# jolibrain/jolineedle

Hardware: AMD Instinct MI355X
Metric: glimpse-patches/sec (448px, seq-len 20) REINFORCE step (higher is better)
Workload: dtype f32; 1 GPU; configs[2]/[3]: REINFORCE rollout, gpt-nano + yolox-nano encoder, 448px, seq-len 20, --enable-stop, 64 agents/GPU x 1 GPU, 4480x4480 synthetic images, forced non-STOP actions (S=T); global_batch=64, seq_len=20

## Files before the change

jolineedle_amd/csrc/api_net.hip:

```cpp
#include <algorithm>
#include <cstring>

#include "jn_internal.h"

using namespace jnr;

extern "C"
__global__ void bn_eval_table_kernel(const float* __restrict__ gamma, const float* __restrict__ beta,
                                     const float* __restrict__ rmean, const float* __restrict__ rvar, ChanTab t0,
                                     ChanTab t1, int C, float eps) {
  const int c = blockIdx.x * blockDim.x + threadIdx.x;
  if (c >= C) return;
  const float sc = gamma[c] / sqrtf(rvar[c] + eps);
  const float sh = beta[c] - rmean[c] * sc;
  t0.sc[c] = sc; t0.sh[c] = sh; t0.fl[c] = 1.0f;
  if (t1.sc) { t1.sc[c] = sc; t1.sh[c] = sh; t1.fl[c] = 1.0f; }
}

extern "C"
__global__ void fill_kernel(float* p, float v, long long n) {
  const long long i = (long long)blockIdx.x * blockDim.x + threadIdx.x;
  if (i < n) p[i] = v;
}

// ... 16 lines not shown
static bool defer_tab_runs(const Net& net, const View& v, int N, ChanTab& t) {
  const int off = net.tab_off[v.buf] + v.coff;
  auto deferred = [&](int c) { return net.h_td_hw[off + c] > 0.0f && (double)N * net.h_td_hw[off + c] <= (double)JN_DEFER_MAX_M; };
  bool any = false;
  for (int c = 0; c < v.C && !any; ++c) any = deferred(c);
  if (!any) return false;
  int ns = 0;
  bool fits = true;
  for (int c = 0; c < v.C && fits;) {
    const int tc = off + c;
    const bool d = deferred(c);
    int e = c + 1;
    if (d) {
      while (e < v.C && net.h_td_src[off + e] == net.h_td_src[tc] + (e - c) && net.h_td_goff[off + e] == net.h_td_goff[tc] + (e - c) &&
             net.h_td_boff[off + e] == net.h_td_boff[tc] + (e - c) && net.h_td_hw[off + e] == net.h_td_hw[tc])
        ++e;
    } else {
      while (e < v.C && !deferred(e)) ++e;
    }
    if (ns == 4) { fits = false; break; }
    const ChanTab::Run run{c, e, d ? net.h_td_src[tc] : -1, net.h_td_goff[tc], net.h_td_boff[tc], net.h_td_hw[tc]};
    (ns == 0 ? t.r0 : ns == 1 ? t.r1 : ns == 2 ? t.r2 : t.r3) = run;
    ++ns;
    c = e;
  }
  t.nseg = fits ? ns : 0;
  return true;
}

static inline float* slot_save(const Net& net, int slot) { return net.save + (size_t)slot * 2 * net.stat_channels; }

StemSrc patch_src(const void* ptr, int P, long long sample_stride) {
  return StemSrc{ptr, nullptr, sample_stride ? sample_stride : 3LL * P * P, (long long)P * P, P};
}

int ensure_slots(jn_ctx* ctx, Net& net, int n_slots) {
  if (net.n_slots >= n_slots) return JN_OK;
  const int MB = ctx->cfg.max_batch;
  float *tab = nullptr, *save = nullptr;
  double* stats = nullptr;
  char* act = nullptr;
  int rc;
  if ((rc = dev_alloc(ctx, &act, (size_t)n_slots * net.per_image_floats * MB * act_esz(net)))) return rc;
  if ((rc = dev_alloc(ctx, &tab, (size_t)n_slots * 3 * net.tab_channels))) return rc;
  if ((rc = dev_alloc(ctx, &save, (size_t)n_slots * 2 * net.stat_channels))) return rc;
  if ((rc = dev_alloc(ctx, &stats, (size_t)n_slots * JN_NREP * 2 * net.stat_channels))) return rc;
  const int n_old = net.n_slots;
  if (n_old > 0) {
    JN_HIP(hipDeviceSynchronize());
    JN_HIP(hipMemcpy(act, net.act, (size_t)n_old * net.per_image_floats * MB * act_esz(net), hipMemcpyDeviceToDevice));
    JN_HIP(hipMemcpy(tab, net.tab, (size_t)n_old * 3 * net.tab_channels * sizeof(float), hipMemcpyDeviceToDevice));
    JN_HIP(hipMemcpy(save, net.save, (size_t)n_old * 2 * net.stat_channels * sizeof(float), hipMemcpyDeviceToDevice));
    JN_HIP(hipMemcpy(stats, net.stats, (size_t)n_old * JN_NREP * 2 * net.stat_channels * sizeof(double), hipMemcpyDeviceToDevice));
  }
  net.act = act; net.tab = tab; net.save = save; net.stats = stats; net.n_slots = n_slots;
  for (int sl = n_old; sl < n_slots; ++sl) {
    float* t = tab + (size_t)sl * 3 * net.tab_channels;
    const long long n = net.tab_channels;
    hipLaunchKernelGGL(fill_kernel, dim3((unsigned)((n + 255) / 256)), dim3(256), 0, 0, t, 1.0f, n);
    hipLaunchKernelGGL(fill_kernel, dim3((unsigned)((2 * n + 255) / 256)), dim3(256), 0, 0, t + n, 0.0f, 2 * n);
  }
  JN_HIP(hipGetLastError());
  JN_HIP(hipDeviceSynchronize());
  if (n_old == 0) net.eval_tab_dirty = true;
  return JN_OK;
}

int refresh_eval_table(jn_ctx* ctx, Net& net, hipStream_t s) {
  if (!net.eval_tab_dirty) return JN_OK;
  for (const Op& op : net.ops) {
    if (op.wslot < 0) continue;
    const ConvW& cw = net.convs[op.wslot];
    if (!cw.has_bn) continue;
    ChanTab t1{nullptr, nullptr, nullptr};
    if (op.alias.buf >= 0) t1 = view_tab(net, 0, op.alias);
    hipLaunchKernelGGL(bn_eval_table_kernel, dim3((cw.cout + 63) / 64), dim3(64), 0, s, cw.gamma_dev, cw.beta_dev,
                       cw.rmean_dev, cw.rvar_dev, view_tab(net, 0, op.out), t1, cw.cout, kBnEps);
  }
  JN_HIP(hipGetLastError());
  net.eval_tab_dirty = false;
  return JN_OK;
}

static void refresh_x3_planes(jn_ctx* ctx, Net& net, hipStream_t s) {
  if (net.x3_hi == 0) {
    size_t lo = ctx->arena_size, hi = 0;
    for (const Op& op : net.ops) {
      if (op.kind != OP_PW || op.wslot < 0) continue;
      const ConvW& cw = net.convs[op.wslot];
      if (!cw.w_dev) continue;
      const size_t o = (size_t)(cw.w_dev - ctx->params);
      lo = std::min(lo, o); hi = std::max(hi, o + (size_t)cw.cout * cw.cin);
    }
    net.x3_lo = lo / 8 * 8; net.x3_hi = hi > lo ? (hi + 7) / 8 * 8 : 0;
  }
  if (net.x3_hi > net.x3_lo && net.x3_dirty) {
    launch_w_split3(ctx->params + net.x3_lo, ctx->params_x3 + 3 * net.x3_lo, (long long)(net.x3_hi - net.x3_lo), s);
    net.x3_dirty = false;
  }
}

void mark_params_written(jn_ctx* ctx) {
  for (Net& net : ctx->nets) net.eval_tab_dirty = net.x3_dirty = true;
}

static View net_full_view(const Net& net, int buf) {
  View v; v.buf = buf; v.H = net.bufs[buf].H; v.W = net.bufs[buf].W; v.C = net.bufs[buf].C; v.coff = 0;
  return v;
}

static int ensure_defer_tables(jn_ctx* ctx, Net& net) {
  if (net.defer_built) return JN_OK;
  net.defer_built = true;
  if (!ctx->params || !defer_eligible(net)) return JN_OK;
  const int n_ops = net.n_backbone_ops < 0 ? (int)net.ops.size() : net.n_backbone_ops;
  const int TC = net.tab_channels, SC = net.stat_channels;
  std::vector<int> td_src(TC, -1), td_g(TC, 0), td_b(TC, 0), fd_g(SC, 0), fd_b(SC, 0), fd_t0(SC, 0), fd_t1(SC, -1);
  std::vector<float> td_hw(TC, 0.0f), fd_hw(SC, 0.0f);
  std::vector<float*> fd_rm(SC, nullptr), fd_rv(SC, nullptr);
  for (int oi = 0; oi < n_ops; ++oi) {
    const Op& op = net.ops[oi];
    if (op.wslot < 0) continue;
    const ConvW& cw = net.convs[op.wslot];
    const float hw = (float)(op.out.H * op.out.W);
    for (int j = 0; j < cw.cout; ++j) {
      const int i = cw.stat_off + j;
      const int g = (int)(cw.gamma_dev - ctx->params) + j, b = (int)(cw.beta_dev - ctx->params) + j;
      fd_hw[i] = hw; fd_g[i] = g; fd_b[i] = b; fd_rm[i] = cw.rmean_dev + j; fd_rv[i] = cw.rvar_dev + j;
      const View* vs[2] = {&op.out, op.alias.buf >= 0 ? &op.alias : nullptr};
      for (int k = 0; k < 2; ++k) {
        if (!vs[k]) continue;
        const int tc = net.tab_off[vs[k]->buf] + vs[k]->coff + j;
        (k == 0 ? fd_t0 : fd_t1)[i] = tc;
        td_src[tc] = i; td_hw[tc] = hw; td_g[tc] = g; td_b[tc] = b;
      }
    }
  }
  int rc;
  auto up = [&](auto** dst, const auto& host) -> int {
    using T = typename std::remove_reference<decltype(host[0])>::type;
    typename std::remove_const<T>::type* d = nullptr;
    if ((rc = dev_alloc(ctx, &d, host.size()))) return rc;
    JN_HIP(hipMemcpy(d, host.data(), host.size() * sizeof(T), hipMemcpyHostToDevice));
    *dst = d;
    return JN_OK;
  };
  if ((rc = up(&net.td_src, td_src)) || (rc = up(&net.td_goff, td_g)) || (rc = up(&net.td_boff, td_b)) || (rc = up(&net.td_hw, td_hw)) ||
      (rc = up(&net.fd_hw, fd_hw)) || (rc = up(&net.fd_goff, fd_g)) || (rc = up(&net.fd_boff, fd_b)) || (rc = up(&net.fd_t0, fd_t0)) ||
      (rc = up(&net.fd_t1, fd_t1)) || (rc = up(&net.fd_rm, fd_rm)) || (rc = up(&net.fd_rv, fd_rv)))
    return rc;
  net.h_td_hw.assign(TC, 0.0f);
  for (int tc = 0; tc < TC; ++tc) if (td_src[tc] >= 0) net.h_td_hw[tc] = td_hw[tc];
  net.h_td_src = td_src; net.h_td_goff = td_g; net.h_td_boff = td_b;
  net.defer_ok = true;
  return JN_OK;
}

namespace {
struct OpProfile {
  std::vector<hipEvent_t> ev;
  hipStream_t s;
  double tot_us = 0, tot_b = 0;
  OpProfile(bool on, int n_events, hipStream_t s_) : s(s_) {
    if (on) { ev.resize(n_events); for (auto& e : ev) (void)hipEventCreate(&e); }
  }
  ~OpProfile() { for (auto& e : ev) (void)hipEventDestroy(e); }
  explicit operator bool() const { return !ev.empty(); }
  void mark(int i) { if (!ev.empty()) (void)hipEventRecord(ev[i], s); }
  void row(const Op& op, int from, int to, double bytes, bool bwd) {
    static const char* kn[] = {"stem", "pw", "dw", "conv3", "spp", "upsample", "addact", "pred"};
    float ms = 0;
    (void)hipEventElapsedTime(&ms, ev[from], ev[to]);
    tot_us += ms * 1e3; tot_b += bytes;
    fprintf(stderr, "%-8s %-44s in %3dx%3dx%3d out %3dx%3dx%3d s%d", kn[op.kind], op.name.c_str(), op.in.H, op.in.W, op.in.C,
            op.out.H, op.out.W, op.out.C, op.stride);
    if (bwd) fprintf(stderr, " acc %d  %8.1f us  %8.1f MB  %6.0f GB/s\n", (int)op.acc_in, ms * 1e3, bytes / 1e6, bytes / (ms * 1e-3) / 1e9);
    else fprintf(stderr, "  %8.1f us  %7.1f MB  %7.0f GB/s\n", ms * 1e3, bytes / 1e6, bytes / (ms * 1e-3) / 1e9);
  }
  void total() { fprintf(stderr, "# total %.1f us, %.1f MB, %.0f GB/s\n", tot_us, tot_b / 1e6, tot_b / (tot_us * 1e-6) / 1e9); }
};
}

static void invalidate_slot_state(jn_ctx* ctx, int ni, int slot) {
  if (ni == ctx->enc_net) {
    if (slot == 0) ctx->sup_valid = false;
    else if (ni != JN_NET_DETECTOR || slot < det_slot_base(ctx)) ctx->train_out_valid = false;
  }
  if (ni == JN_NET_DETECTOR && slot >= det_slot_base(ctx) && slot - det_slot_base(ctx) < (int)ctx->det_pass.size())
    ctx->det_pass[slot - det_slot_base(ctx)].valid = false;
}

int run_net(jn_ctx* ctx, int ni, int N, const StemSrc& ss, int slot, int train, const int* skip_flag, int skip_when,
            hipStream_t s, bool with_head, int first_op) {
  Net& net = ctx->nets[ni];
  const int MB = ctx->cfg.max_batch;
  int rc;
  invalidate_slot_state(ctx, ni, slot);
  if (!train && (rc = refresh_eval_table(ctx, net, s))) return rc;
  const bool x3 = ctx->params_x3 && !std::getenv("JN_NO_PW_X3");
  if (x3) refresh_x3_planes(ctx, net, s);
  double* stats = train ? slot_stats(net, slot) : nullptr;
  float* save = train ? slot_save(net, slot) : nullptr;
  if (train && !ctx->stats_prezeroed) JN_HIP(hipMemsetAsync(stats, 0, (size_t)JN_NREP * 2 * net.stat_channels * sizeof(double), s));
  const long long rep_stride = 2LL * net.stat_channels;
  if (train && !with_head && (rc = ensure_defer_tables(ctx, net))) return rc;
  const bool defer = train && !with_head && net.defer_ok;
  std::vector<FwdStep> plan;
  if ((rc = plan_forward(net, N, train != 0, with_head, first_op, defer, plan))) return rc;
  const int n_ops = first_op + (int)plan.size();
  auto ptr = [&](const View& v) { return view_ptr(net, slot, MB, v); };
  auto tab = [&](const View& v) {
    ChanTab t = view_tab(net, slot, v);
    if (defer && defer_tab_runs(net, v, N, t)) {
      const int off = net.tab_off[v.buf] + v.coff;
      t.dsrc = net.td_src + off; t.dhw = net.td_hw + off; t.dgoff = net.td_goff + off; t.dboff = net.td_boff + off;
      t.dparams = ctx->params; t.dstats = stats; t.drep_stride = rep_stride; t.dN = N; t.dmax = JN_DEFER_MAX_M;
    }
    return t;
  };
  auto ld = [&](const View& v) { return net.bufs[v.buf].C; };
  auto finalize = [&](const Op& op, const ConvW& cw, bool deferred) {
    if (!train || !cw.has_bn || deferred) return;
    ChanTab t1{nullptr, nullptr, nullptr};
    if (op.alias.buf >= 0) t1 = tab(op.alias);
    launch_bn_finalize(stats + 2 * cw.stat_off, rep_stride, (double)N * op.out.H * op.out.W, cw.gamma_dev, cw.beta_dev,
                       defer ? nullptr : cw.rmean_dev, defer ? nullptr : cw.rvar_dev, defer ? nullptr : save + 2 * cw.stat_off,
                       tab(op.out), t1, cw.cout, kBnEps, kBnMomentum, skip_flag, skip_when, s);
  };
  static const bool layer_profile = std::getenv("JN_LAYER_PROFILE") != nullptr;
  OpProfile prof(layer_profile, n_ops + 1, s);
  prof.mark(first_op);
  std::vector<char> up_done(n_ops, 0);
  for (int oi = first_op; oi < n_ops; ++oi) {
    const Op& op = net.ops[oi];
    const FwdStep& st = plan[oi - first_op];
    switch (st.route) {
      case FR_STEM: {
        const ConvW& cw = net.convs[op.wslot];
        StemArgs a{ss.src, ss.positions, ss.pos_stride, ss.sample_stride, ss.chan_stride, ss.row_stride, net.P, N, cw.cout,
                   cw.w_dev, ptr(op.out), ld(op.out), net.act_dtype, train ? stats + 2 * cw.stat_off : nullptr, rep_stride,
                   skip_flag, skip_when, st.deferred ? JN_NREP_DEFER : JN_NREP, ss.src_u8};
        launch_stem(a, s);
        finalize(op, cw, st.deferred);
        break;
      }
      case FR_DWPW:
      case FR_DWPW_ADD: {
        const Op& nx = net.ops[st.link];
        DwPwArgs f{};
        f.in = ptr(op.in); f.in_ld = ld(op.in); f.itab = tab(op.in); f.w_dw = net.convs[op.wslot].w_dev; f.mtab = tab(op.out);
        f.w_pw = net.convs[nx.wslot].w_dev; f.out = ptr(nx.out); f.out_ld = ld(nx.out); f.dtype = net.act_dtype;
        f.C = op.out.C; f.cout = nx.out.C; f.N = N; f.H = op.in.H; f.W = op.in.W; f.OH = op.out.H; f.OW = op.out.W;
        f.stride = op.stride; f.skip_flag = skip_flag; f.skip_when = skip_when;
        if (st.route == FR_DWPW_ADD) {
          const Op& ad = net.ops[st.add];
          f.res = ptr(ad.res); f.res_ld = ld(ad.res); f.rtab = tab(ad.res); f.ptab = tab(nx.out);
          f.out = ptr(ad.out); f.out_ld = ld(ad.out);
        }
        launch_dwpw(f, s);
        break;
      }
      case FR_CONV: {
        const ConvW& cw = net.convs[op.wslot];
        ConvArgs a{};
        a.in = ptr(op.in); a.in_ld = ld(op.in); a.in_dtype = net.act_dtype; a.itab = tab(op.in); a.w = cw.w_dev;
        a.w_bf16 = cw.w_bf16;
        if (x3 && op.kind == OP_PW && (cw.w_dev - ctx->params) % 8 == 0) a.w_x3 = ctx->params_x3 + 3 * (cw.w_dev - ctx->params);
        a.bias = cw.b_dev; a.out = ptr(op.out); a.out_ld = ld(op.out); a.out_dtype = net.act_dtype;
        a.bf16_mfma = net.act_dtype == JN_BF16;
        a.N = N; a.H = op.in.H; a.W = op.in.W; a.OH = op.out.H; a.OW = op.out.W;
        a.cin = op.in.C; a.cout = op.out.C; a.stride = op.stride; a.act = op.act;
        a.stats = (train && cw.has_bn) ? stats + 2 * cw.stat_off : nullptr;
        a.stats_rep_stride = rep_stride;
        a.stats_nrep = st.deferred ? JN_NREP_DEFER : JN_NREP;
        a.skip_flag = skip_flag; a.skip_when = skip_when;
        if (st.link >= 0 && pw_fused_upsample_supported(a)) {
          const Op& up = net.ops[st.link];
          a.up_out = ptr(up.out); a.up_ld = ld(up.out); up_done[st.link] = 1;
        }
        if (op.kind == OP_PW) { JN_CHECK(launch_pw(a, s) == 0, JN_ESTATE, "1x1 conv %s: no kernel for this shape", op.name.c_str()); }
        else if (op.kind == OP_DW) launch_dw(a, s); else launch_conv3(a, s);
        finalize(op, cw, st.deferred);
        break;
// ... 420 lines not shown
```

jolineedle_amd/csrc/jn_internal.h:

```cpp
#pragma once
#include <hip/hip_runtime.h>

#include <cstdint>
#include <cstdio>
#include <map>
#include <string>
#include <vector>

#include "../../include/jnroll.h"
#include "jn_kernels.h"

namespace jnr {

void set_error(const char* fmt, ...);

#define JN_HIP(call)                                                                      \
  do {                                                                                    \
    hipError_t e_ = (call);                                                               \
    if (e_ != hipSuccess) {                                                               \
      jnr::set_error("%s failed: %s (%s:%d)", #call, hipGetErrorString(e_), __FILE__, __LINE__); \
      return JN_EHIP;                                                                     \
    }                                                                                     \
  } while (0)

#define JN_CHECK(cond, code, ...)   \
  do {                              \
    if (!(cond)) {                  \
      jnr::set_error(__VA_ARGS__);   \
      return (code);                \
    }                               \
  } while (0)

struct Buf {
  int H = 0, W = 0, C = 0;
  size_t per_image() const { return (size_t)H * W * C; }
};

struct View {
  int buf = -1;
  int H = 0, W = 0;
  int C = 0;
  int coff = 0;
};

enum OpKind {
  OP_STEM = 0,
  OP_PW,
  OP_DW,
  OP_CONV3,
  OP_SPP,
  OP_UPSAMPLE,
  OP_ADDACT,
  OP_PRED,
};

struct Op {
  OpKind kind;
  View in, out;
  View res;
  View alias;
  int stride = 1;
  int act = ACT_SILU;
  int wslot = -1;
  int level = 0, anchor0 = 0;
  bool acc_in = false;
  bool acc_res = false;
  std::string name;
};

struct ConvW {
  std::string prefix;
  std::string prefix2;
  int cout_first = 0;
  int cin = 0, cout = 0, k = 1, groups = 1;
  bool has_bn = true;
  bool has_bias = false;
  float* w_dev = nullptr;
  void* w_bf16 = nullptr;
  float* b_dev = nullptr;
  float *gamma_dev = nullptr, *beta_dev = nullptr;
  float *rmean_dev = nullptr, *rvar_dev = nullptr;
  int stat_off = 0;
};

struct Net {
  std::string prefix;
  bool depthwise = false;
  float depth = 0, width = 0;
  int P = 0;
  std::vector<Buf> bufs;
  std::vector<Op> ops;
  std::vector<ConvW> convs;
  View fpn[3];
  int n_backbone_ops = -1;
  size_t x3_lo = 0, x3_hi = 0;
  bool x3_dirty = true;
  int n_anchors = 0, head_hid = 0;
  float* pred_w[3] = {nullptr, nullptr, nullptr};
  float* pred_b[3] = {nullptr, nullptr, nullptr};
  size_t per_image_floats = 0;
  std::vector<size_t> buf_off;
  std::vector<int> tab_off;
  int tab_channels = 0;
  int stat_channels = 0;
  int n_slots = 0;
  int act_dtype = 0;
  char* act = nullptr;
  float* tab = nullptr;
  float* save = nullptr;
  double* stats = nullptr;
  int g_slots = 0;
  float* gact = nullptr;
  double* bred = nullptr;
  float* bconsts = nullptr;
  bool eval_tab_dirty = true;
  bool defer_ok = false, defer_built = false;
  int *td_src = nullptr, *td_goff = nullptr, *td_boff = nullptr; float* td_hw = nullptr;
  float* fd_hw = nullptr; int *fd_goff = nullptr, *fd_boff = nullptr, *fd_t0 = nullptr, *fd_t1 = nullptr;
  float **fd_rm = nullptr, **fd_rv = nullptr;
  std::vector<float> h_td_hw;
  std::vector<int> h_td_src, h_td_goff, h_td_boff;
};

enum BwdRoute {
  BR_NONE = 0,
  BR_PW_FUSED, BR_PW_FUSED_HALVES,
  BR_DW_FUSED, BR_STEM_FUSED,
  BR_PW, BR_DW, BR_STEM, BR_CONV3_S1, BR_CONV3_S2,
  BR_ADDACT_COPY, BR_ADDACT_FOLD,
  BR_SPP, BR_UPSAMPLE,
};
struct BwdStep {
  BwdRoute route = BR_NONE;
  View g;
  int red_by = 0;
  int red_in = -1, red_half = -1, red_in2 = -1, red_half2 = -1, red_split = 0;
  bool red2 = false;
  int fold = -1;
};
int plan_backward(const Net& net, bool with_head, int fpn_zero, std::vector<BwdStep>& plan);

enum FwdRoute {
  FR_NONE = 0,
  FR_STEM, FR_CONV,
  FR_DWPW, FR_DWPW_ADD,
  FR_ABSORBED,
  FR_SPP, FR_UPSAMPLE, FR_ADDACT, FR_PRED,
};
struct FwdStep {
  FwdRoute route = FR_NONE;
  int link = -1;
  int add = -1;
  bool deferred = false;
};
bool defer_eligible(const Net& net);
int plan_forward(const Net& net, int N, bool train, bool with_head, int first_op, bool defer, std::vector<FwdStep>& plan);

struct ParamEntry {
  jn_param_info info;
};
void add_param(std::vector<ParamEntry>& params, const std::string& name, std::initializer_list<int64_t> shape, int dtype,
               bool buffer, bool used);

struct ParamSeg {
  std::string name;
  int kind = 0, d0 = 0, d1 = 0, d2 = 0;
  size_t off = 0, numel = 0;
};

struct GptW {
  float *wte = nullptr, *wpe = nullptr, *embed_class = nullptr;
  float *proj_wt = nullptr, *proj_b = nullptr;
  float *pos1d = nullptr;
  float *pos2d_col = nullptr, *pos2d_row = nullptr;
  float *efpn_w = nullptr;
  float *efpn_lin_wt = nullptr, *efpn_lin_b = nullptr;
  float *head_wt = nullptr;
  float *lnf_w = nullptr, *lnf_b = nullptr;
  struct Layer {
// ... 175 lines not shown
```

jolineedle_amd/csrc/jn_kernels.h:

```cpp
#pragma once
#include <hip/hip_runtime.h>

#include <cstdint>

#include "../../include/jnroll.h"

namespace jnr {

enum { ACT_NONE = 0, ACT_SILU = 1, ACT_RELU = 2, ACT_SIGMOID = 3 };
enum { JN_F32 = 0, JN_BF16 = 1 };

constexpr int JN_NREP = 32;
constexpr int JN_WPART_MAX = 16384;

struct ChanTab {
  float* sc; float* sh; float* fl;
  const int* dsrc;
  const float* dhw;
  const int* dgoff; const int* dboff;
  const float* dparams;
  const double* dstats;
  long long drep_stride;
  int dN;
  long long dmax;
  struct Run { int c0, c1, stat0, g0, b0; float hw; };
  int nseg;
  Run r0, r1, r2, r3;
};
constexpr long long JN_DEFER_MAX_M = 65536;
constexpr int JN_NREP_DEFER = 8;

struct SlotBatch {
  int n = 1;
  long long act = 0;
  long long grad = 0;
  long long tab = 0;
  long long save = 0;
  long long red = 0;
  long long consts = 0;
  long long pos = 0;
};

struct StemArgs {
  const void* src; const int64_t* positions; int pos_stride;
  long long sample_stride, chan_stride; int row_stride;
  int P, N, cout;
  const float* w; void* out; int out_ld; int out_dtype;
  double* stats;
  long long stats_rep_stride;
  const int* skip_flag; int skip_when;
  int stats_nrep;
  int src_u8;
};

struct ConvArgs {
  const void* in; int in_ld; int in_dtype; ChanTab itab;
  const float* w; const float* bias;
  const void* w_bf16;
  void* out; int out_ld; int out_dtype;
  int bf16_mfma;
  int N, H, W, OH, OW, cin, cout, stride, act;
  int accumulate;
  int w_transposed;
  int in_identity;
  double* stats; long long stats_rep_stride;
  int stats_nrep;
  const int* skip_flag; int skip_when;
  int n_slots;
  long long in_slot_stride, out_slot_stride, tab_slot_stride;
  const void* w_x3;
  void* up_out; int up_ld;
};

struct DwPwArgs {
  const void* in; int in_ld; ChanTab itab; const float* w_dw; ChanTab mtab; const float* w_pw;
  void* out; int out_ld; int dtype; int C, cout, N, H, W, OH, OW, stride;
  const int* skip_flag; int skip_when;
  const void* res; int res_ld; ChanTab rtab;
  ChanTab ptab;
};
bool dwpw_supported(int C, int cout, int stride);
int launch_dwpw(const DwPwArgs& a, hipStream_t s);
int launch_stem(const StemArgs& a, hipStream_t s);
bool stem_rows_aligned(const StemArgs& a);
int launch_dw(const ConvArgs& a, hipStream_t s);
int launch_pw(const ConvArgs& a, hipStream_t s);
bool pw_fused_upsample_supported(const ConvArgs& a);
bool pw_res_supported(const ConvArgs& a);
int launch_pw_dir(const ConvArgs& a, int ctw, hipStream_t s);
int launch_pw_wide(const ConvArgs& a, hipStream_t s);
bool pw_xs_supported(const ConvArgs& a);
int launch_pw_xs(const ConvArgs& a, int pt, hipStream_t s, int wg_per_cu = 0);
int launch_pw_x3(const ConvArgs& a, int pt, hipStream_t s, int wg_per_cu = 0);
bool pw_x3_preferred(const ConvArgs& a);
bool pw_x3_bwd_data_supported(int cout, int cin);
int launch_pw_x3_bwd_data(const ConvArgs& a, const float* w, void* w3t, hipStream_t s);
bool pw_x1_supported(const ConvArgs& a);
int launch_pw_x1(const ConvArgs& a, hipStream_t s);
void launch_w_split3(const float* w, void* w3, long long n_floats, hipStream_t s);
int launch_spp(void* cat, int dtype, int ld, int h, int H, int W, int N, ChanTab it, const int* skip_flag,
               int skip_when, hipStream_t s);
int launch_upsample(const void* in, int in_ld, void* out, int out_ld, int dtype, int C, int H, int W, int N,
                    const int* skip_flag, int skip_when, hipStream_t s);
int launch_addact(const void* z, int z_ld, ChanTab zt, const void* res, int res_ld, ChanTab rt, void* out, int out_ld,
                  int dtype, int C, long long M, const int* skip_flag, int skip_when, hipStream_t s);
int launch_bn_finalize(const double* stats, long long rep_stride, double count, const float* gamma, const float* beta, float* run_mean,
                       float* run_var, float* save, ChanTab t0, ChanTab t1, int C, float eps, float momentum,
                       const int* skip_flag, int skip_when, hipStream_t s);
struct BnAllArgs {
  const double* stats; long long rep_stride; int n_stat; int N;
  const float* hw;
  const int* goff; const int* boff;
  const float* params;
  const int* t0; const int* t1;
  float* tab; int tab_channels;
  float* save;
  float* const* run_mean; float* const* run_var;
  float eps, momentum;
  const int* skip_flag; int skip_when;
  long long defer_max_m;
};
int launch_bn_finalize_all(const BnAllArgs& a, hipStream_t s);
int launch_nhwc_to_nchw(const void* in, int dtype, int in_ld, ChanTab it, float* out, int C, int HW, int N,
                        hipStream_t s);
int launch_efpn_linear(const float* e, const float* wt, float* part, int N, int K, int Co, int KS,
                       const int* skip_flag, int skip_when, hipStream_t s);

int launch_conv3(const ConvArgs& a, hipStream_t s);
int launch_conv3_bwd_data_s2(const float* gz, int g_ld, const float* w, float* gin, int gin_ld, int H, int W, int OH,
                             int OW, int Co, int Ci, int N, int accumulate, hipStream_t s,
                             const SlotBatch& sb = SlotBatch{});
int launch_conv3_bwd_weight(const float* gz, int g_ld, const void* x, int x_dtype, int x_ld, ChanTab it, float* gw, int H,
                            int W, int OH, int OW, int Co, int Ci, int N, int stride, hipStream_t s,
                            const SlotBatch& sb = SlotBatch{});
int launch_head_pred(const void* reg, int reg_ld, ChanTab rt, const void* cls, int cls_ld, ChanTab ct, int dtype,
                     const float* wp, const float* bp, float* raw, int hid, int Hl, int Wl, int stride, int A, int a0,
                     int N, hipStream_t s, int logits_only = 0);
int launch_det_scatter(const float* boxes, const int* counts, float* out_boxes, int* out_counts, int B, int cols, int col,
                       int K, const int* skip_flag, int skip_when, hipStream_t s);
int launch_postprocess(const float* raw, int A, int N, float conf, float nms_thr, float clamp_max, float* boxes,
                       int* counts, int max_out, int* stats, hipStream_t s);

struct DetGeom { int A; int a0[3]; int H[3]; int W[3]; int stride[3]; };
int launch_yolox_loss(const float* raw, const float* labels, int N, int nb, const DetGeom& geo, float* d_raw, float* acc,
                      int use_l1, float loss_scale, float* metrics, float* scale, hipStream_t s);
int launch_head_pred_bwd(const float* d_raw, const float* scale, const void* reg, int reg_ld, ChanTab rt, const void* cls,
                         int cls_ld, ChanTab ct, int dtype, const float* wp, float* g_reg, float* g_cls, float* g_wp,
                         float* g_bp, int hid, int HW, int A, int a0, int N, hipStream_t s);

int launch_bn_bwd_reduce(const float* g, int g_ld, const void* z, int z_dtype, int z_ld, ChanTab t, const float* save,
                         int C, long long M, double* red_out, long long rep_stride, hipStream_t s,
                         const SlotBatch& sb = SlotBatch{});
int launch_bn_bwd_consts(const double* red, long long rep_stride, double count, const float* gamma, const float* beta,
                         const float* save, float* consts, float* g_gamma, float* g_beta, int C, hipStream_t s,
                         const SlotBatch& sb = SlotBatch{}, int raw_moment = 0);
int launch_bn_bwd_gz(float* g, int g_ld, const void* z, int z_dtype, int z_ld, ChanTab t, const float* save,
                     const float* consts, int C, long long M, hipStream_t s, const SlotBatch& sb = SlotBatch{});
int launch_pw_bwd_weight(const float* gz, int g_ld, const void* x, int x_dtype, int x_ld, ChanTab it, float* gw,
                         float* wpart, long long M, int N, int K, hipStream_t s, const SlotBatch& sb = SlotBatch{},
                         long long gz_slot_stride = -1);
int launch_wpart_reduce(float* gw, float* wpart, int n, hipStream_t s);
struct PwBwdFusedArgs {
  const float* g; int g_ld;
  const float* z; int z_ld; ChanTab ot;
  const float* save; const float* consts;
  const float* x; int x_ld; ChanTab it;
  const float* w;
  float* gx; int gx_ld; int accumulate;
  float* gw; float* wpart;
  long long M; int cout, cin;
  SlotBatch sb;
  double* red_in; long long red_rep_stride; double* red_in2; int red_split;
  const float* gadd; int gadd_ld;
  const float* red2_z; int red2_ld; const float* red2_sc; const float* red2_sh;
};
struct DwBwdFusedArgs {
// ... 181 lines not shown
```

jolineedle_amd/csrc/kernels_pwxs.hip:

```cpp
#include <hip/hip_runtime.h>

#include <algorithm>
#include <cstdlib>

#include "jn_kernels.h"
#include "jn_reduce.h"
#include "jn_tab.h"
#include "jn_types.h"

namespace jnr {

struct UpsDst { float* out; int ld; int W; int HW; };
template <bool UPS>
__device__ __forceinline__ void ups_store(const UpsDst& u, long long m, int n, const f32x4& v) {
  if constexpr (UPS) {
    const long long img = m / u.HW;
    const int rem = (int)(m - img * u.HW), y = rem / u.W, x = rem - y * u.W;
    float* d = u.out + ((img * 2 * (u.HW / u.W) + 2 * y) * (2LL * u.W) + 2 * x) * u.ld + n;
    *reinterpret_cast<f32x4*>(d) = v;
    *reinterpret_cast<f32x4*>(d + u.ld) = v;
    d += 2LL * u.W * u.ld;
    *reinterpret_cast<f32x4*>(d) = v;
    *reinterpret_cast<f32x4*>(d + u.ld) = v;
  }
// ... 134 lines not shown
static void launch_pw_xs_t(const ConvArgs& a, long long M, int wg_per_cu, hipStream_t s) {
  constexpr int BM = 16 * PT;
  const size_t smem = ((size_t)BM * (K + 8) + 3 * K) * sizeof(float);
  auto kern = pw_xs_kernel<K, CTW, PT, D, UPS>;
  static int places = 0;
  if (!places) {
    (void)hipFuncSetAttribute(reinterpret_cast<const void*>(kern), hipFuncAttributeMaxDynamicSharedMemorySize, 160 * 1024);
    int per_cu = 0;
    if (hipOccupancyMaxActiveBlocksPerMultiprocessor(&per_cu, reinterpret_cast<const void*>(kern), 256, smem) != hipSuccess || per_cu < 1) per_cu = 1;
    places = per_cu;
  }
  const long long n_tiles = (M + BM - 1) / BM;
  const int per_cu = std::max(1, std::min(places, wg_per_cu > 0 ? wg_per_cu : 2));
  const long long gx = std::min<long long>(n_tiles, 256LL * per_cu);
  hipLaunchKernelGGL(kern, dim3((unsigned)gx), dim3(256), smem, s, (const float*)a.in, a.in_ld, a.itab, a.w, (float*)a.out,
                     a.out_ld, M, a.stats, a.stats_rep_stride, a.stats_nrep > 0 ? a.stats_nrep : JN_NREP, a.skip_flag,
                     a.skip_when, UpsDst{(float*)a.up_out, a.up_ld, a.W, a.H * a.W});
}

bool pw_xs_supported(const ConvArgs& a) {
  if (a.bf16_mfma || a.in_dtype != JN_F32 || a.out_dtype != JN_F32 || a.bias || a.act != ACT_NONE || a.w_transposed ||
      a.accumulate || a.n_slots > 1)
    return false;
  const int K = a.cin, N = a.cout;
  if (!(K == 64 || K == 128 || K == 256 || K == 512) || !(N == 64 || N == 128 || N == 256)) return false;
  if (K == 64 && N == 256) return false;
  if (K == 512 && N != 256) return false;
  if (K == 256 && N == 64) return false;
  return a.in_ld % 4 == 0 && a.out_ld % 4 == 0;
}

int launch_pw_xs(const ConvArgs& a, int pt, hipStream_t s, int wg_per_cu) {
  if (!pw_xs_supported(a)) return -1;
  const long long M = (long long)a.N * a.H * a.W;
  const int K = a.cin, ctw = a.cout / 64;
  if (pt == 0) {
    const bool big = K == 512 || (K == 64 && ctw == 2);
    pt = big ? 4 : 2;
    if (wg_per_cu == 0) wg_per_cu = big ? 1 : 2;
  }
  if (a.up_out) {
    if (!(K == 256 && ctw == 2 && pt == 2)) return -1;
    launch_pw_xs_t<256, 2, 2, 4, true>(a, M, wg_per_cu, s);
    return 0;
  }
#define JN_XS(K_, C_, D_)                                                          \
  if (K == K_ && ctw == C_) {                                                      \
    if (pt == 4) launch_pw_xs_t<K_, C_, 4, D_>(a, M, wg_per_cu, s); else launch_pw_xs_t<K_, C_, 2, D_>(a, M, wg_per_cu, s); \
    return 0;                                                                      \
  }
  JN_XS(64, 1, 4) JN_XS(64, 2, 4)
  JN_XS(128, 1, 8) JN_XS(128, 2, 8) JN_XS(128, 4, 2)
  JN_XS(256, 2, 4) JN_XS(256, 4, 2)
  JN_XS(512, 4, 2)
#undef JN_XS
  return -1;
}


__global__ __launch_bounds__(256) void w_split3_kernel(const float* __restrict__ w, bf16_t* __restrict__ w3, long long n8) {
  const long long i = (long long)blockIdx.x * 256 + threadIdx.x;
  if (i >= n8) return;
  const f32x4 a = *reinterpret_cast<const f32x4*>(w + 8 * i), b = *reinterpret_cast<const f32x4*>(w + 8 * i + 4);
  bf16x8 h, m, l;
#pragma unroll
  for (int e = 0; e < 8; ++e) {
    const float v = e < 4 ? a[e] : b[e - 4];
    const bf16_t vh = (bf16_t)v;
    const float r1 = v - (float)vh;
    const bf16_t vm = (bf16_t)r1;
    const float r2 = r1 - (float)vm;
    h[e] = vh; m[e] = vm; l[e] = (bf16_t)r2;
  }
  bf16x8* o = reinterpret_cast<bf16x8*>(w3 + 24 * i);
  o[0] = h; o[1] = m; o[2] = l;
}

void launch_w_split3(const float* w, void* w3, long long n_floats, hipStream_t s) {
  const long long n8 = n_floats / 8;
  if (n8 <= 0) return;
  hipLaunchKernelGGL(w_split3_kernel, dim3((unsigned)((n8 + 255) / 256)), dim3(256), 0, s, w, (bf16_t*)w3, n8);
}

struct SlotSpan { int n_slots; long long in, out; };
template <int K, int CTW, int PT, int D, int NP, typename XT, bool UPS = false, bool SLOTS = false>
__global__ __launch_bounds__(256, (K <= 64 ? 3 : CTW <= 2 ? 2 : 1)) void pw_x3_kernel(
    const XT* __restrict__ x, int x_ld, ChanTab it, const bf16_t* __restrict__ w3, XT* __restrict__ out, int out_ld,
    long long M, double* __restrict__ stats, long long rep_stride, int nrep, const int* __restrict__ skip_flag,
    int skip_when, UpsDst ups, SlotSpan sl) {
  if (skip_flag && *skip_flag >= skip_when) return;
  constexpr int BM = 16 * PT, LDK = K + 16, KQ = K / 4, NJ = K / 32, N = 64 * CTW;
  constexpr int NX = BM * KQ / 256;
  constexpr int NXB = NX < 16 ? NX : 16;
  static_assert(256 % KQ == 0 && NX >= 1 && NX % NXB == 0 && NJ % D == 0, "pw_x3 tile mapping");
  extern __shared__ __attribute__((aligned(16))) unsigned char smem_raw[];
  bf16_t* Xp = reinterpret_cast<bf16_t*>(smem_raw);
  float* Tb = reinterpret_cast<float*>(Xp + NP * BM * LDK);
  const int tid = threadIdx.x, lane = tid & 63, wave = tid >> 6;
  const int lm = lane & 15, g = lane >> 4;
  const long long tiles_per_slot = (M + BM - 1) / BM;
  const long long n_tiles = SLOTS ? tiles_per_slot * sl.n_slots : tiles_per_slot;

  const bf16_t* wrow[CTW];
#pragma unroll
  for (int c = 0; c < CTW; ++c)
    wrow[c] = SLOTS ? w3 + (long long)(wave * CTW + c) * (K / 32) * 3 * 512 + lane * 8
                    : w3 + ((long long)((wave * CTW + c) * 16 + lm) * (K / 8) + g) * 24;
  auto wfrag = [&](int c, int j, int t) -> bf16x8 {
    if constexpr (SLOTS) return *reinterpret_cast<const bf16x8*>(wrow[c] + (j * 3 + t) * 512);
    else return *reinterpret_cast<const bf16x8*>(wrow[c] + 96 * j + 8 * t);
  };
  bf16x8 wr[D][CTW][NP];
#pragma unroll
  for (int u = 0; u < D; ++u)
#pragma unroll
    for (int c = 0; c < CTW; ++c)
#pragma unroll
      for (int t = 0; t < NP; ++t) wr[u][c][t] = wfrag(c, u, t);

  const int q = tid % KQ, r0 = tid / KQ;
  constexpr int RS = 256 / KQ;
  f32x4 xr[NXB];
  const XT* xs = x;
  auto fetch = [&](long long m0, int b) {
#pragma unroll
    for (int u = 0; u < NXB; ++u) {
      long long m = m0 + r0 + (long long)(b * NXB + u) * RS;
      m = m < M ? m : M - 1;
      xr[u] = ld4(xs + m * x_ld + 4 * q);
    }
  };
  auto locate = [&](long long t) -> long long {
    if constexpr (SLOTS) {
      const long long slot = t / tiles_per_slot;
      xs = x + slot * sl.in;
      return (t - slot * tiles_per_slot) * BM;
    } else {
      return t * BM;
    }
  };
  long long tile = blockIdx.x;
  long long m0 = locate(tile);
  fetch(m0, 0);
  tab_to_lds(Tb, K, K, it, tid, 256);
  __syncthreads();
  const f32x4 sc = *reinterpret_cast<const f32x4*>(Tb + 4 * q), sh = *reinterpret_cast<const f32x4*>(Tb + K + 4 * q),
              fl = *reinterpret_cast<const f32x4*>(Tb + 2 * K + 4 * q);
  f32x4 s1[CTW], s2[CTW];
#pragma unroll
  for (int c = 0; c < CTW; ++c) { s1[c] = f32x4{0.f, 0.f, 0.f, 0.f}; s2[c] = s1[c]; }

#pragma unroll 1
  for (; tile < n_tiles; tile += gridDim.x) {
    XT* outs = out;
    if constexpr (SLOTS) outs = out + (tile / tiles_per_slot) * sl.out;
#pragma unroll
    for (int b = 0; b < NX / NXB; ++b) {
      if (b > 0) fetch(m0, b);
#pragma unroll
      for (int u = 0; u < NXB; ++u) {
        const int r = r0 + (b * NXB + u) * RS;
        f32x4 v = tf4_tab(xr[u], sc, sh, fl);
        if (m0 + r >= M) v = f32x4{0.f, 0.f, 0.f, 0.f};
        const bf16x4 vh = __builtin_convertvector(v, bf16x4);
        bf16_t* dst = Xp + r * LDK + 4 * q;
        *reinterpret_cast<bf16x4*>(dst) = vh;
        if constexpr (NP == 3) {
          const f32x4 r1 = v - __builtin_convertvector(vh, f32x4);
          const bf16x4 vm = __builtin_convertvector(r1, bf16x4);
          const f32x4 r2 = r1 - __builtin_convertvector(vm, f32x4);
          const bf16x4 vl = __builtin_convertvector(r2, bf16x4);
          *reinterpret_cast<bf16x4*>(dst + BM * LDK) = vm;
          *reinterpret_cast<bf16x4*>(dst + 2 * BM * LDK) = vl;
        }
      }
    }
    __syncthreads();
    const long long m0_this = m0;
    if (tile + gridDim.x < n_tiles) { m0 = locate(tile + gridDim.x); fetch(m0, 0); }

    f32x4 acc[CTW][PT];
#pragma unroll
    for (int c = 0; c < CTW; ++c)
#pragma unroll
      for (int p = 0; p < PT; ++p) acc[c][p] = f32x4{0.f, 0.f, 0.f, 0.f};
    const bf16_t* xrow = Xp + lm * LDK + 8 * g;
#pragma unroll 1
    for (int j0 = 0; j0 < NJ; j0 += D) {
#pragma unroll
      for (int u = 0; u < D; ++u) {
        const int j = j0 + u;
        bf16x8 xa[PT][NP], wa[CTW][NP];
#pragma unroll
        for (int p = 0; p < PT; ++p)
#pragma unroll
          for (int t = 0; t < NP; ++t) xa[p][t] = *reinterpret_cast<const bf16x8*>(xrow + t * BM * LDK + p * 16 * LDK + 32 * j);
#pragma unroll
        for (int c = 0; c < CTW; ++c)
#pragma unroll
          for (int t = 0; t < NP; ++t) wa[c][t] = wr[u][c][t];
        if constexpr (D < NJ) {
          const int jn = j + D < NJ ? j + D : j + D - NJ;
#pragma unroll
          for (int c = 0; c < CTW; ++c)
#pragma unroll
            for (int t = 0; t < NP; ++t) wr[u][c][t] = wfrag(c, jn, t);
          __builtin_amdgcn_sched_barrier(0);
        }
        constexpr int TW[6] = {2, 0, 1, 1, 0, 0}, TX[6] = {0, 2, 1, 0, 1, 0};
#pragma unroll
        for (int e = (NP == 3 ? 0 : 5); e < 6; ++e)
#pragma unroll
          for (int c = 0; c < CTW; ++c)
#pragma unroll
            for (int p = 0; p < PT; ++p)
              acc[c][p] = __builtin_amdgcn_mfma_f32_16x16x32_bf16(wa[c][TW[e]], xa[p][TX[e]], acc[c][p], 0, 0, 0);
      }
    }

#pragma unroll
    for (int c = 0; c < CTW; ++c) {
      const int n = (wave * CTW + c) * 16 + 4 * g;
#pragma unroll
      for (int p = 0; p < PT; ++p) {
        const long long m = m0_this + 16 * p + lm;
        const f32x4 v = acc[c][p];
        if (m < M) { st4(outs + m * out_ld + n, v); ups_store<UPS>(ups, m, n, v); }
        s1[c] += v; s2[c] += v * v;
      }
    }
    __syncthreads();
  }

  if (stats) {
    float* red = Tb;
    if constexpr (3 * K < 2 * N) red = reinterpret_cast<float*>(Xp);
#pragma unroll
    for (int c = 0; c < CTW; ++c) {
      const int n = (wave * CTW + c) * 16 + 4 * g;
#pragma unroll
      for (int r = 0; r < 4; ++r) {
        const float a = row16_sum(s1[c][r]);
        const float b = row16_sum(s2[c][r]);
        if (lm == 0) { red[2 * (n + r)] = a; red[2 * (n + r) + 1] = b; }
      }
    }
    __syncthreads();
    double* st = stats + (blockIdx.x % nrep) * rep_stride;
    for (int i = tid; i < 2 * N; i += 256) atomicAdd(st + i, (double)red[i]);
  }
}

template <int K, int CTW, int PT, int D, int NP, typename XT, bool UPS = false, bool SLOTS = false>
static void launch_pw_x3_t(const ConvArgs& a, long long M, int wg_per_cu, hipStream_t s) {
  constexpr int BM = 16 * PT;
  const size_t smem = (size_t)NP * BM * (K + 16) * sizeof(bf16_t) + 3 * K * sizeof(float);
  auto kern = pw_x3_kernel<K, CTW, PT, D, NP, XT, UPS, SLOTS>;
  static int places = 0;
  if (!places) {
    (void)hipFuncSetAttribute(reinterpret_cast<const void*>(kern), hipFuncAttributeMaxDynamicSharedMemorySize, 160 * 1024);
    int per_cu = 0;
    if (hipOccupancyMaxActiveBlocksPerMultiprocessor(&per_cu, reinterpret_cast<const void*>(kern), 256, smem) != hipSuccess || per_cu < 1) per_cu = 1;
    places = per_cu;
  }
  const int n_slots = SLOTS ? std::max(1, a.n_slots) : 1;
  const long long n_tiles = (M + BM - 1) / BM * n_slots;
  const int per_cu = std::max(1, std::min(places, wg_per_cu > 0 ? wg_per_cu : 2));
  const long long gx = std::min<long long>(n_tiles, 256LL * per_cu);
  hipLaunchKernelGGL(kern, dim3((unsigned)gx), dim3(256), smem, s, (const XT*)a.in, a.in_ld, a.itab, (const bf16_t*)a.w_x3,
                     (XT*)a.out, a.out_ld, M, a.stats, a.stats_rep_stride, a.stats_nrep > 0 ? a.stats_nrep : JN_NREP,
                     a.skip_flag, a.skip_when, UpsDst{(float*)a.up_out, a.up_ld, a.W, a.H * a.W},
                     SlotSpan{n_slots, a.in_slot_stride, a.out_slot_stride});
}

static bool pw_xs_shape(int K, int N) {
  if (!(K == 64 || K == 128 || K == 256 || K == 512) || !(N == 64 || N == 128 || N == 256)) return false;
  return !(K == 64 && N == 256) && !(K == 512 && N != 256) && !(K == 256 && N == 64);
}

bool pw_x3_preferred(const ConvArgs& a) {
  if (!a.w_x3 || !pw_xs_supported(a)) return false;
  const int K = a.cin, N = a.cout;
  return (K == 64 && (N == 64 || N == 128)) || (K == 128 && (N == 64 || N == 128)) || (K == 256 && N == 256);
}

bool pw_x1_supported(const ConvArgs& a) {
  return a.w_x3 && a.bf16_mfma && a.in_dtype == JN_BF16 && a.out_dtype == JN_BF16 && !a.bias && a.act == ACT_NONE && !a.w_transposed &&
         !a.accumulate && a.n_slots <= 1 && pw_xs_shape(a.cin, a.cout) && a.in_ld % 4 == 0 && a.out_ld % 4 == 0;
}

int launch_pw_x1(const ConvArgs& a, hipStream_t s) {
  if (!pw_x1_supported(a)) return -1;
  const long long M = (long long)a.N * a.H * a.W;
  const int K = a.cin, ctw = a.cout / 64;
  const int wg = (K == 512 || ctw == 4) ? 1 : 2;
#define JN_X1(K_, C_, P_, D_) if (K == K_ && ctw == C_) { launch_pw_x3_t<K_, C_, P_, D_, 1, bf16_t>(a, M, wg, s); return 0; }
  JN_X1(64, 1, 2, 2) JN_X1(64, 2, 2, 2) JN_X1(128, 1, 2, 4) JN_X1(128, 2, 2, 4) JN_X1(128, 4, 2, 4)
  JN_X1(256, 2, 4, 2) JN_X1(256, 4, 4, 2) JN_X1(512, 4, 4, 2)
#undef JN_X1
  return -1;
}

int launch_pw_x3(const ConvArgs& a, int pt, hipStream_t s, int wg_per_cu) {
  if (!pw_xs_supported(a) || !a.w_x3) return -1;
  const long long M = (long long)a.N * a.H * a.W;
  const int K = a.cin, ctw = a.cout / 64;
  if (pt == 0) {
    pt = K == 256 ? 4 : 2;
    if (wg_per_cu == 0) wg_per_cu = (K == 256 || (K == 64 && ctw == 2) || (K == 128 && ctw == 2 && M <= 16384)) ? 1 : 2;
  }
  if (a.up_out) {
    if (!(K == 128 && ctw == 1 && pt == 2)) return -1;
    launch_pw_x3_t<128, 1, 2, 4, 3, float, true>(a, M, wg_per_cu, s);
    return 0;
  }
#define JN_X3(K_, C_, P_, D_) if (K == K_ && ctw == C_ && pt == P_) { launch_pw_x3_t<K_, C_, P_, D_, 3, float>(a, M, wg_per_cu, s); return 0; }
  JN_X3(64, 1, 2, 2) JN_X3(64, 2, 2, 2) JN_X3(128, 1, 2, 4) JN_X3(128, 2, 2, 4) JN_X3(256, 4, 4, 2)
#ifdef JN_X3_ALL_SHAPES
  JN_X3(64, 1, 4, 2) JN_X3(64, 2, 4, 2) JN_X3(128, 1, 4, 4) JN_X3(128, 2, 4, 4) JN_X3(128, 4, 2, 2) JN_X3(128, 4, 4, 2)
  JN_X3(256, 2, 2, 2) JN_X3(256, 2, 4, 2) JN_X3(256, 4, 2, 2) JN_X3(512, 4, 2, 2)
#endif
#undef JN_X3
  return -1;
}

__global__ __launch_bounds__(256) void w_split3_t_kernel(const float* __restrict__ w, bf16_t* __restrict__ w3t, int cout, int cin) {
  const int i = blockIdx.x * 256 + threadIdx.x;
  const int groups = cout / 8;
  if (i >= cin * groups) return;
  const int n = i % cin, gq = i / cin;
  const int NJ = cout / 32, j = gq >> 2, g = gq & 3;
  bf16x8 h, m, l;
#pragma unroll
  for (int e = 0; e < 8; ++e) {
    const float v = w[(long long)(8 * gq + e) * cin + n];
    const bf16_t vh = (bf16_t)v;
    const float r1 = v - (float)vh;
    const bf16_t vm = (bf16_t)r1;
    const float r2 = r1 - (float)vm;
    h[e] = vh; m[e] = vm; l[e] = (bf16_t)r2;
  }
  bf16_t* o = w3t + ((long long)((n >> 4) * NJ + j) * 3 * 64 + g * 16 + (n & 15)) * 8;
  *reinterpret_cast<bf16x8*>(o) = h;
  *reinterpret_cast<bf16x8*>(o + 512) = m;
  *reinterpret_cast<bf16x8*>(o + 1024) = l;
}

bool pw_x3_bwd_data_supported(int cout, int cin) {
  return (cout == 256 && (cin == 128 || cin == 256 || cin == 512)) || (cout == 128 && cin == 256);
}

int launch_pw_x3_bwd_data(const ConvArgs& a, const float* w, void* w3t, hipStream_t s) {
  const int K = a.cin, N = a.cout;
  if (!pw_x3_bwd_data_supported(K, N) || a.accumulate || a.in_dtype != JN_F32 || a.out_dtype != JN_F32 || a.bias ||
      a.act != ACT_NONE || a.in_ld % 4 != 0 || a.out_ld % 4 != 0 || a.stats)
    return -1;
  hipLaunchKernelGGL(w_split3_t_kernel, dim3((unsigned)((N * (K / 8) + 255) / 256)), dim3(256), 0, s, w, (bf16_t*)w3t, K, N);
  const long long M = (long long)a.N * a.H * a.W;
  ConvArgs b = a;
  b.w_x3 = w3t; b.up_out = nullptr;
  if (K == 256 && N == 128) { launch_pw_x3_t<256, 2, 2, 2, 3, float, false, true>(b, M, 2, s); return 0; }
  if (K == 128 && N == 256) { launch_pw_x3_t<128, 4, 2, 4, 3, float, false, true>(b, M, 2, s); return 0; }
  for (int n0 = 0; n0 < N; n0 += 256) {
    b.w_x3 = (const bf16_t*)w3t + (long long)n0 * K * 3;
    b.out = (float*)a.out + n0;
    launch_pw_x3_t<256, 4, 2, 2, 3, float, false, true>(b, M, 2, s);
  }
  return 0;
}

}
```

Baseline: 12910 glimpse-patches/s.

## Store pointwise-conv split-bf16 weights in MFMA fragment order and widen x3 shape coverage

Adds a kernel that writes the three bf16 planes of eligible pointwise conv weights in MFMA fragment order, so each lane loads a contiguous bf16x8 per fragment instead of a strided gather. The pw_x3 kernel gains a FRAG template flag that selects this layout. The preferred x3 path is also extended to more shapes (128->256, 256->128, 512->256, plus an upsample variant for 256->128). This adds an extra weight-split launch whenever parameters change. The fragment writes overwrite the row-order planes in the same buffer, so any other consumer of those planes would read the wrong layout.

```diff
diff --git a/jolineedle_amd/csrc/api_net.hip b/jolineedle_amd/csrc/api_net.hip
--- a/jolineedle_amd/csrc/api_net.hip
+++ b/jolineedle_amd/csrc/api_net.hip
@@ -122,22 +122,37 @@
   return JN_OK;
 }
 
-static void refresh_x3_planes(jn_ctx* ctx, Net& net, hipStream_t s) {
+static int refresh_x3_planes(jn_ctx* ctx, Net& net, hipStream_t s) {
   if (net.x3_hi == 0) {
     size_t lo = ctx->arena_size, hi = 0;
+    std::vector<X3FragConv> frag;
     for (const Op& op : net.ops) {
       if (op.kind != OP_PW || op.wslot < 0) continue;
       const ConvW& cw = net.convs[op.wslot];
       if (!cw.w_dev) continue;
       const size_t o = (size_t)(cw.w_dev - ctx->params);
       lo = std::min(lo, o); hi = std::max(hi, o + (size_t)cw.cout * cw.cin);
+      if (o % 8 == 0 && op.in.C * op.out.C == cw.cin * cw.cout && pw_x3_fragment_order(op.in.C, op.out.C)) {
+        bool seen = false;
+        for (const X3FragConv& f : frag) seen = seen || f.off == (long long)o;
+        if (!seen) frag.push_back(X3FragConv{(long long)o, op.out.C, op.in.C});
+      }
+    }
+    if (!frag.empty() && !net.x3_frag) {
+      int rc;
+      if ((rc = dev_alloc(ctx, &net.x3_frag, frag.size()))) return rc;
+      JN_HIP(hipMemcpy(net.x3_frag, frag.data(), frag.size() * sizeof(X3FragConv), hipMemcpyHostToDevice));
+      net.x3_frag_n = (int)frag.size();
+      for (const X3FragConv& f : frag) net.x3_frag_max = std::max(net.x3_frag_max, f.cout * f.cin);
     }
     net.x3_lo = lo / 8 * 8; net.x3_hi = hi > lo ? (hi + 7) / 8 * 8 : 0;
   }
   if (net.x3_hi > net.x3_lo && net.x3_dirty) {
     launch_w_split3(ctx->params + net.x3_lo, ctx->params_x3 + 3 * net.x3_lo, (long long)(net.x3_hi - net.x3_lo), s);
+    launch_w_split3_frag(ctx->params, ctx->params_x3, net.x3_frag, net.x3_frag_n, net.x3_frag_max, s);
     net.x3_dirty = false;
   }
+  return JN_OK;
 }
 
 void mark_params_written(jn_ctx* ctx) {
@@ -238,7 +253,7 @@
   invalidate_slot_state(ctx, ni, slot);
   if (!train && (rc = refresh_eval_table(ctx, net, s))) return rc;
   const bool x3 = ctx->params_x3 && !std::getenv("JN_NO_PW_X3");
-  if (x3) refresh_x3_planes(ctx, net, s);
+  if (x3 && (rc = refresh_x3_planes(ctx, net, s))) return rc;
   double* stats = train ? slot_stats(net, slot) : nullptr;
   float* save = train ? slot_save(net, slot) : nullptr;
   if (train && !ctx->stats_prezeroed) JN_HIP(hipMemsetAsync(stats, 0, (size_t)JN_NREP * 2 * net.stat_channels * sizeof(double), s));
diff --git a/jolineedle_amd/csrc/jn_internal.h b/jolineedle_amd/csrc/jn_internal.h
--- a/jolineedle_amd/csrc/jn_internal.h
+++ b/jolineedle_amd/csrc/jn_internal.h
@@ -95,6 +95,8 @@
   int n_backbone_ops = -1;
   size_t x3_lo = 0, x3_hi = 0;
   bool x3_dirty = true;
+  X3FragConv* x3_frag = nullptr;
+  int x3_frag_n = 0, x3_frag_max = 0;
   int n_anchors = 0, head_hid = 0;
   float* pred_w[3] = {nullptr, nullptr, nullptr};
   float* pred_b[3] = {nullptr, nullptr, nullptr};
diff --git a/jolineedle_amd/csrc/jn_kernels.h b/jolineedle_amd/csrc/jn_kernels.h
--- a/jolineedle_amd/csrc/jn_kernels.h
+++ b/jolineedle_amd/csrc/jn_kernels.h
@@ -91,7 +91,13 @@
 int launch_pw_wide(const ConvArgs& a, hipStream_t s);
 bool pw_xs_supported(const ConvArgs& a);
 int launch_pw_xs(const ConvArgs& a, int pt, hipStream_t s, int wg_per_cu = 0);
-int launch_pw_x3(const ConvArgs& a, int pt, hipStream_t s, int wg_per_cu = 0);
+int launch_pw_x3(const ConvArgs& a, int pt, hipStream_t s, int wg_per_cu = 0, int frag = -1);
+constexpr bool pw_x3_fragment_order(int cin, int cout) {
+  return (cin == 64 && (cout == 64 || cout == 128)) || (cin == 128 && (cout == 64 || cout == 128 || cout == 256)) ||
+         (cin == 256 && (cout == 128 || cout == 256)) || (cin == 512 && cout == 256);
+}
+struct X3FragConv { long long off; int cout, cin; };
+void launch_w_split3_frag(const float* params, void* params_x3, const X3FragConv* tab, int n_convs, int max_weights, hipStream_t s);
 bool pw_x3_preferred(const ConvArgs& a);
 bool pw_x3_bwd_data_supported(int cout, int cin);
 int launch_pw_x3_bwd_data(const ConvArgs& a, const float* w, void* w3t, hipStream_t s);
diff --git a/jolineedle_amd/csrc/kernels_pwxs.hip b/jolineedle_amd/csrc/kernels_pwxs.hip
--- a/jolineedle_amd/csrc/kernels_pwxs.hip
+++ b/jolineedle_amd/csrc/kernels_pwxs.hip
@@ -240,8 +240,38 @@
   hipLaunchKernelGGL(w_split3_kernel, dim3((unsigned)((n8 + 255) / 256)), dim3(256), 0, s, w, (bf16_t*)w3, n8);
 }
 
+__global__ __launch_bounds__(256) void w_split3_frag_kernel(const float* __restrict__ params, bf16_t* __restrict__ params_x3,
+                                                            const X3FragConv* __restrict__ tab) {
+  const X3FragConv c = tab[blockIdx.y];
+  const int i = blockIdx.x * 256 + threadIdx.x, groups = c.cin / 8;
+  if (i >= c.cout * groups) return;
+  const int n = i / groups, kq = i - n * groups, j = kq >> 2, g = kq & 3;
+  const float* w = params + c.off + 8LL * i;
+  const f32x4 a = *reinterpret_cast<const f32x4*>(w), b = *reinterpret_cast<const f32x4*>(w + 4);
+  bf16x8 h, m, l;
+#pragma unroll
+  for (int e = 0; e < 8; ++e) {
+    const float v = e < 4 ? a[e] : b[e - 4];
+    const bf16_t vh = (bf16_t)v;
+    const float r1 = v - (float)vh;
+    const bf16_t vm = (bf16_t)r1;
+    const float r2 = r1 - (float)vm;
+    h[e] = vh; m[e] = vm; l[e] = (bf16_t)r2;
+  }
+  bf16_t* o = params_x3 + 3 * c.off + ((long long)((n >> 4) * (c.cin / 32) + j) * 3 * 64 + g * 16 + (n & 15)) * 8;
+  *reinterpret_cast<bf16x8*>(o) = h;
+  *reinterpret_cast<bf16x8*>(o + 512) = m;
+  *reinterpret_cast<bf16x8*>(o + 1024) = l;
+}
+
+void launch_w_split3_frag(const float* params, void* params_x3, const X3FragConv* tab, int n_convs, int max_weights, hipStream_t s) {
+  if (n_convs <= 0 || max_weights <= 0) return;
+  hipLaunchKernelGGL(w_split3_frag_kernel, dim3((unsigned)((max_weights / 8 + 255) / 256), (unsigned)n_convs), dim3(256), 0, s,
+                     params, (bf16_t*)params_x3, tab);
+}
+
 struct SlotSpan { int n_slots; long long in, out; };
-template <int K, int CTW, int PT, int D, int NP, typename XT, bool UPS = false, bool SLOTS = false>
+template <int K, int CTW, int PT, int D, int NP, typename XT, bool UPS = false, bool SLOTS = false, bool FRAG = SLOTS>
 __global__ __launch_bounds__(256, (K <= 64 ? 3 : CTW <= 2 ? 2 : 1)) void pw_x3_kernel(
     const XT* __restrict__ x, int x_ld, ChanTab it, const bf16_t* __restrict__ w3, XT* __restrict__ out, int out_ld,
     long long M, double* __restrict__ stats, long long rep_stride, int nrep, const int* __restrict__ skip_flag,
@@ -262,10 +292,10 @@
   const bf16_t* wrow[CTW];
 #pragma unroll
   for (int c = 0; c < CTW; ++c)
-    wrow[c] = SLOTS ? w3 + (long long)(wave * CTW + c) * (K / 32) * 3 * 512 + lane * 8
-                    : w3 + ((long long)((wave * CTW + c) * 16 + lm) * (K / 8) + g) * 24;
+    wrow[c] = FRAG ? w3 + (long long)(wave * CTW + c) * (K / 32) * 3 * 512 + lane * 8
+                   : w3 + ((long long)((wave * CTW + c) * 16 + lm) * (K / 8) + g) * 24;
   auto wfrag = [&](int c, int j, int t) -> bf16x8 {
-    if constexpr (SLOTS) return *reinterpret_cast<const bf16x8*>(wrow[c] + (j * 3 + t) * 512);
+    if constexpr (FRAG) return *reinterpret_cast<const bf16x8*>(wrow[c] + (j * 3 + t) * 512);
     else return *reinterpret_cast<const bf16x8*>(wrow[c] + 96 * j + 8 * t);
   };
   bf16x8 wr[D][CTW][NP];
@@ -409,11 +439,11 @@
   }
 }
 
-template <int K, int CTW, int PT, int D, int NP, typename XT, bool UPS = false, bool SLOTS = false>
+template <int K, int CTW, int PT, int D, int NP, typename XT, bool UPS = false, bool SLOTS = false, bool FRAG = SLOTS>
 static void launch_pw_x3_t(const ConvArgs& a, long long M, int wg_per_cu, hipStream_t s) {
   constexpr int BM = 16 * PT;
   const size_t smem = (size_t)NP * BM * (K + 16) * sizeof(bf16_t) + 3 * K * sizeof(float);
-  auto kern = pw_x3_kernel<K, CTW, PT, D, NP, XT, UPS, SLOTS>;
+  auto kern = pw_x3_kernel<K, CTW, PT, D, NP, XT, UPS, SLOTS, FRAG>;
   static int places = 0;
   if (!places) {
     (void)hipFuncSetAttribute(reinterpret_cast<const void*>(kern), hipFuncAttributeMaxDynamicSharedMemorySize, 160 * 1024);
@@ -438,8 +468,7 @@
 
 bool pw_x3_preferred(const ConvArgs& a) {
   if (!a.w_x3 || !pw_xs_supported(a)) return false;
-  const int K = a.cin, N = a.cout;
-  return (K == 64 && (N == 64 || N == 128)) || (K == 128 && (N == 64 || N == 128)) || (K == 256 && N == 256);
+  return pw_x3_fragment_order(a.cin, a.cout);
 }
 
 bool pw_x1_supported(const ConvArgs& a) {
@@ -452,31 +481,50 @@
   const long long M = (long long)a.N * a.H * a.W;
   const int K = a.cin, ctw = a.cout / 64;
   const int wg = (K == 512 || ctw == 4) ? 1 : 2;
-#define JN_X1(K_, C_, P_, D_) if (K == K_ && ctw == C_) { launch_pw_x3_t<K_, C_, P_, D_, 1, bf16_t>(a, M, wg, s); return 0; }
+#define JN_X1(K_, C_, P_, D_) \
+  if (K == K_ && ctw == C_) { launch_pw_x3_t<K_, C_, P_, D_, 1, bf16_t, false, false, pw_x3_fragment_order(K_, 64 * C_)>(a, M, wg, s); return 0; }
   JN_X1(64, 1, 2, 2) JN_X1(64, 2, 2, 2) JN_X1(128, 1, 2, 4) JN_X1(128, 2, 2, 4) JN_X1(128, 4, 2, 4)
   JN_X1(256, 2, 4, 2) JN_X1(256, 4, 4, 2) JN_X1(512, 4, 4, 2)
 #undef JN_X1
   return -1;
 }
 
-int launch_pw_x3(const ConvArgs& a, int pt, hipStream_t s, int wg_per_cu) {
+int launch_pw_x3(const ConvArgs& a, int pt, hipStream_t s, int wg_per_cu, int frag) {
   if (!pw_xs_supported(a) || !a.w_x3) return -1;
   const long long M = (long long)a.N * a.H * a.W;
   const int K = a.cin, ctw = a.cout / 64;
+  const int rule = pw_x3_fragment_order(K, a.cout) ? 1 : 0;
+  if (frag < 0) frag = rule;
   if (pt == 0) {
-    pt = K == 256 ? 4 : 2;
-    if (wg_per_cu == 0) wg_per_cu = (K == 256 || (K == 64 && ctw == 2) || (K == 128 && ctw == 2 && M <= 16384)) ? 1 : 2;
+    const bool sq256 = K == 256 && ctw == 4;
+    pt = sq256 ? 4 : 2;
+    if (wg_per_cu == 0) wg_per_cu = (sq256 || (K == 64 && ctw == 2) || (K == 128 && ctw == 2 && M <= 16384)) ? 1 : 2;
   }
   if (a.up_out) {
-    if (!(K == 128 && ctw == 1 && pt == 2)) return -1;
-    launch_pw_x3_t<128, 1, 2, 4, 3, float, true>(a, M, wg_per_cu, s);
-    return 0;
-  }
-#define JN_X3(K_, C_, P_, D_) if (K == K_ && ctw == C_ && pt == P_) { launch_pw_x3_t<K_, C_, P_, D_, 3, float>(a, M, wg_per_cu, s); return 0; }
-  JN_X3(64, 1, 2, 2) JN_X3(64, 2, 2, 2) JN_X3(128, 1, 2, 4) JN_X3(128, 2, 2, 4) JN_X3(256, 4, 4, 2)
+    if (pt != 2 || frag != rule) return -1;
+    if (K == 128 && ctw == 1) { launch_pw_x3_t<128, 1, 2, 4, 3, float, true, false, pw_x3_fragment_order(128, 64)>(a, M, wg_per_cu, s); return 0; }
+    if (K == 256 && ctw == 2) { launch_pw_x3_t<256, 2, 2, 2, 3, float, true, false, pw_x3_fragment_order(256, 128)>(a, M, wg_per_cu, s); return 0; }
+    return -1;
+  }
 #ifdef JN_X3_ALL_SHAPES
-  JN_X3(64, 1, 4, 2) JN_X3(64, 2, 4, 2) JN_X3(128, 1, 4, 4) JN_X3(128, 2, 4, 4) JN_X3(128, 4, 2, 2) JN_X3(128, 4, 4, 2)
-  JN_X3(256, 2, 2, 2) JN_X3(256, 2, 4, 2) JN_X3(256, 4, 2, 2) JN_X3(512, 4, 2, 2)
+#define JN_X3(K_, C_, P_, D_)                                                                   \
+  if (K == K_ && ctw == C_ && pt == P_) {                                                       \
+    if (frag) launch_pw_x3_t<K_, C_, P_, D_, 3, float, false, false, true>(a, M, wg_per_cu, s);  \
+    else launch_pw_x3_t<K_, C_, P_, D_, 3, float, false, false, false>(a, M, wg_per_cu, s);      \
+    return 0;                                                                                   \
+  }
+#else
+#define JN_X3(K_, C_, P_, D_)                                                                                           \
+  if (K == K_ && ctw == C_ && pt == P_ && frag == rule) {                                                               \
+    launch_pw_x3_t<K_, C_, P_, D_, 3, float, false, false, pw_x3_fragment_order(K_, 64 * C_)>(a, M, wg_per_cu, s);       \
+    return 0;                                                                                                           \
+  }
+#endif
+  JN_X3(64, 1, 2, 2) JN_X3(64, 2, 2, 2) JN_X3(128, 1, 2, 4) JN_X3(128, 2, 2, 4) JN_X3(128, 4, 2, 2)
+  JN_X3(256, 2, 2, 2) JN_X3(256, 4, 4, 2) JN_X3(512, 4, 2, 2)
+#ifdef JN_X3_ALL_SHAPES
+  JN_X3(64, 1, 4, 2) JN_X3(64, 2, 4, 2) JN_X3(128, 1, 4, 4) JN_X3(128, 2, 4, 4) JN_X3(128, 4, 4, 2)
+  JN_X3(256, 2, 4, 2) JN_X3(256, 4, 2, 2)
 #endif
 #undef JN_X3
   return -1;
```

Result: faster. 13090 glimpse-patches/s, median of 6 (+1.4%).
